# o1-labs/proof-systems

Hardware: AMD Instinct MI355X
Metric: MSM Mscalar/s at 2^20 (Vesta) (higher is better)
Workload: dtype u29x9 / u32x8 (255-bit Montgomery integers); 1 GPU; msm_2^20_vesta_srs; points_per_gpu=1048576, points_total=1048576, bases=SRS::<Vesta>::create, scalars=uniform 254-bit, seed 1234+rank, parallelism=point-range x1, world_size_seen=1

## Files before the change

proof_systems_amd/csrc/msm.hip:

```cpp
#include <hip/hip_ext.h>
#include <math.h>
#include "common.hpp"
#include "env.hpp"
#include "curve.cuh"
#include "coop.cuh"
#include "field29.cuh"
#include "host_ec.hpp"
#include "msm.hpp"
#include <condition_variable>
#include <functional>
#include <memory>
#include <thread>

namespace kh {

#define KH_HIGH_PRIO() __builtin_amdgcn_s_setprio(3)

class HostHelper {
    std::thread th_; std::mutex m_; std::condition_variable cv_, done_cv_;
    std::function<void()> job_; bool has_job_ = false, busy_ = false, stop_ = false;
    void loop() {
        std::unique_lock<std::mutex> lk(m_);
        for (;;) {
            cv_.wait(lk, [&] { return has_job_ || stop_; });
// ... 328 lines not shown
        for (int u = 0; u < 8; u++) {
            const u32 b = (u32)(v[u] < 0 ? -v[u] : v[u]) - 1u;
            const u32 pos = lds_inc_agg(cur, b >> PART_LOW, v[u] != 0);
            if (v[u]) mid[pos] = ((b & ((1u << PART_LOW) - 1u)) << 25) | (v[u] < 0 ? 1u << 24 : 0u) | (w << 20) | i;
            i += PART_T;
            while (i >= n) { i -= n; w++; }
        }
    }
}
__global__ void __launch_bounds__(PART_T)
k_part_sort(const u32* __restrict__ mid, const u32* __restrict__ PO, u32 nblk, u32 nb, size_t pt_stride, size_t pt_offset, size_t pt_batch,
            u32 last_group, u32* __restrict__ off, u32* __restrict__ entries) {
    KH_HIGH_PRIO();
    __shared__ u32 hist[1u << PART_LOW], cur[1u << PART_LOW];
    const u32 pidx = blockIdx.x, j = blockIdx.y, tid = threadIdx.x;
    const size_t q = (size_t)j * PART_P + pidx;
    const u32 base = PO[q * nblk], end = PO[(q + 1) * nblk];
    if (tid < (1u << PART_LOW)) hist[tid] = 0;
    __syncthreads();
    for (u32 x0 = base + tid; x0 < end; x0 += 8 * PART_T) {
        u32 m[8];
#pragma unroll
        for (int u = 0; u < 8; u++) { const u32 x = x0 + u * PART_T; m[u] = mid[x < end ? x : end - 1]; }
#pragma unroll
        for (int u = 0; u < 8; u++) (void)lds_inc_agg(hist, m[u] >> 25, x0 + u * PART_T < end);
    }
    __syncthreads();
    if (tid < 64) {
        const u32 a = hist[2 * tid], b = hist[2 * tid + 1];
        u32 inc = a + b;
#pragma unroll
        for (int d = 1; d < 64; d <<= 1) { const u32 o = __shfl_up(inc, d, 64); if (tid >= (u32)d) inc += o; }
        const u32 ex = base + inc - (a + b);
        u32* o = off + (size_t)j * nb + (size_t)pidx * (1u << PART_LOW);
        o[2 * tid] = ex; o[2 * tid + 1] = ex + a;
        cur[2 * tid] = ex; cur[2 * tid + 1] = ex + a;
        if (tid == 63 && pidx == PART_P - 1 && j == last_group) off[(size_t)(j + 1) * nb] = end;
    }
    __syncthreads();
    const u32 pb0 = (u32)(pt_offset + (size_t)j * pt_batch);
    for (u32 x0 = base + tid; x0 < end; x0 += 8 * PART_T) {
        u32 m[8];
#pragma unroll
        for (int u = 0; u < 8; u++) { const u32 x = x0 + u * PART_T; m[u] = mid[x < end ? x : end - 1]; }
#pragma unroll
        for (int u = 0; u < 8; u++) {
            const bool live = x0 + u * PART_T < end;
            const u32 pos = lds_inc_agg(cur, m[u] >> 25, live);
            if (live) entries[pos] = (pb0 + (u32)(((m[u] >> 20) & 15u) * pt_stride) + (m[u] & 0xfffffu)) | ((m[u] & (1u << 24)) << 7);
        }
    }
}
static constexpr u32 MAX_K = 256;
struct KTab { uint8_t k[48]; };
__device__ __forceinline__ u32 pick_K(u32 total, u32 room, u32 kmin, const KTab& tab, u32 nkeys) {
    u32 K = (total + room - 1) / room;
    u32 lo = kmin;
    if (total && nkeys) {
        const float m = (float)total / (float)nkeys;
        int idx = (int)(4.0f * __log2f(m) + 8.5f);
        idx = idx < 0 ? 0 : (idx > 47 ? 47 : idx);
        if (tab.k[idx]) lo = tab.k[idx];
    }
    return K < lo ? lo : (K > MAX_K ? MAX_K : K);
}
__global__ void k_task_reset(u32* __restrict__ len_hist, u32* __restrict__ big) {
    KH_HIGH_PRIO();
    if (threadIdx.x <= MAX_K) len_hist[threadIdx.x] = 0;
    if (threadIdx.x < 2) big[threadIdx.x] = 0;
}
__global__ void k_ntask(const u32* __restrict__ off, size_t nkeys, u32 room, u32 kmin, KTab ktab, u32* __restrict__ nt, u32* __restrict__ len_hist, u32* __restrict__ handed) {
    KH_HIGH_PRIO();
    __shared__ u32 h[MAX_K + 1];
    if (handed && blockIdx.x == 0 && threadIdx.x == 0) handed[0] = 0;
    for (u32 i = threadIdx.x; i <= MAX_K; i += blockDim.x) h[i] = 0;
    __syncthreads();
    const u32 K = pick_K(off[nkeys], room, kmin, ktab, (u32)nkeys);
    size_t key = (size_t)blockIdx.x * blockDim.x + threadIdx.x;
    if (key <= nkeys) {
        u32 n_t = 0;
        if (key < nkeys) {
            u32 c = off[key + 1] - off[key];
            n_t = (c + K - 1) / K;
            u32 len = n_t ? (c + n_t - 1) / n_t : 0;
            atomicAdd(&h[len], 1u);
        }
        nt[key] = n_t;
    }
    __syncthreads();
    for (u32 i = threadIdx.x; i <= MAX_K; i += blockDim.x) if (h[i]) atomicAdd(&len_hist[i], h[i]);
}
__global__ void __launch_bounds__(320) k_len_starts(const u32* __restrict__ len_hist, u32* __restrict__ cursor) {
    KH_HIGH_PRIO();
    __shared__ u32 h[MAX_K + 1];
    if (threadIdx.x <= MAX_K) h[threadIdx.x] = len_hist[threadIdx.x];
    __syncthreads();
    if (threadIdx.x <= MAX_K) {
        u32 run = 0;
        for (u32 L = threadIdx.x + 1; L <= MAX_K; L++) run += h[L];
        cursor[threadIdx.x] = run;
    }
}
__global__ void __launch_bounds__(1024)
k_len_rank(const u32* __restrict__ off, const u32* __restrict__ nt, size_t nkeys,
           u32* __restrict__ cursor, u32* __restrict__ order, u32* __restrict__ rnt) {
    KH_HIGH_PRIO();
// ... 173 lines not shown
    if (!grid_barrier(sync, 3 * G, abort_dev, abort_host, spin_limit)) return;
    KH_TS(6);
    const u32* o = off + (size_t)j * g.nb + b_lo;
    {
        u32 a[FUSED_C], hh[FUSED_C];
#pragma unroll
        for (int u = 0; u < FUSED_C; u++) { const u32 b = tid + u * FUSED_T, bc = b < g.sub ? b : 0u; a[u] = coh_load(o + bc); hh[u] = coh_load(hout + bc); }
        u32 total2;
        lane_sums(bsums + FUSED_B, G, blk, &base, &total2);
#pragma unroll
        for (int u = 0; u < FUSED_C; u++) { const u32 b = tid + u * FUSED_T; if (b < g.sub) lds[b] = a[u] + hh[u]; }
    }
    run = base + ex2;
#pragma unroll
    for (int i = 0; i < FUSED_KPT; i++) {
        const u32 key = key0 + i;
        if ((u32)i < g.kpt && key <= g.nkeys) toff[key] = run;
        run += nt[i];
    }
    __syncthreads();
    KH_TS(7);
    const u32 pb0 = (u32)(g.pt_offset + (size_t)j * g.pt_batch);
    const u32 e_first = 4 * (q_lo + tid);
    u32 w = e_first / g.n, i = e_first - w * g.n;
#pragma unroll
    for (int t = 0; t < FUSED_V; t++) asm volatile("" : "+v"(dv[t][0]), "+v"(dv[t][1]));
#pragma unroll
    for (int t = 0; t < FUSED_V; t++) {
#pragma unroll
        for (int l = 0; l < 4; l++) {
            const u32 c = (dv[t][l >> 1] >> (16 * (l & 1))) & 0xffffu, b = (c & 0x7fffu) - b_lo;
            if (c != 0xffffu && b < g.sub) {
                u32 ii = i + l, ww = w;
                if (ii >= g.n) { ii -= g.n; ww++; }
                const u32 slot = atomicAdd(&lds[b], 1u);
                entries[slot] = (pb0 + (u32)(ww * g.pt_stride) + ii) | ((c & 0x8000u) << 16);
            }
        }
        i += 4 * FUSED_T;
        while (i >= g.n) { i -= g.n; w++; }
    }
    __syncthreads();
    KH_TS(8);
    if (tid == 0) {
        const u32 out = __hip_atomic_fetch_add(sync + 1, 1u, __ATOMIC_RELAXED, __HIP_MEMORY_SCOPE_AGENT);
        if (out == G - 1) {
            __hip_atomic_store(sync, 0u, __ATOMIC_RELAXED, __HIP_MEMORY_SCOPE_AGENT);
            __hip_atomic_store(sync + 1, 0u, __ATOMIC_RELAXED, __HIP_MEMORY_SCOPE_AGENT);
        }
    }
}
static constexpr u32 PART2_MAXLOW = 11, PART2_MAXPASS = 8;
__global__ void __launch_bounds__(PART_T)
k_part2_scatter(const int32_t* __restrict__ digits, u32 tot_e, u32 nblk, u32 low, const u32* __restrict__ PO, u32* __restrict__ mid, u32* __restrict__ xlist, u32* __restrict__ big) {
    KH_HIGH_PRIO();
    __shared__ u32 cur[PART_P];
    const u32 blk = blockIdx.x, j = blockIdx.y, tid = threadIdx.x;
    if (blk == 0 && j == 0 && tid == 0) { xlist[0] = 0; xlist[1] = 0; big[0] = 0; }
    if (tid < PART_P) cur[tid] = PO[((size_t)j * PART_P + tid) * nblk + blk];
    __syncthreads();
    const u32 e_lo = (u32)((u64)tot_e * blk / nblk), e_hi = (u32)((u64)tot_e * (blk + 1) / nblk);
    const int32_t* d = digits + (size_t)j * tot_e;
    for (u32 e0 = e_lo + tid; e0 < e_hi; e0 += 8 * PART_T) {
        int32_t v[8];
#pragma unroll
        for (int u = 0; u < 8; u++) { const u32 e = e0 + u * PART_T; v[u] = d[e < e_hi ? e : e_hi - 1]; if (e >= e_hi) v[u] = 0; }
#pragma unroll
        for (int u = 0; u < 8; u++) {
            const u32 b = (u32)(v[u] < 0 ? -v[u] : v[u]) - 1u;
            const u32 pos = lds_inc_agg(cur, b & (PART_P - 1u), v[u] != 0);
            if (v[u]) mid[pos] = ((b >> 8) << 17) | (v[u] < 0 ? 1u << 16 : 0u) | (e0 + u * PART_T - e_lo);
        }
    }
}
struct WideTasks { u32 room, kmin, nkeys; KTab ktab; };
__global__ void __launch_bounds__(PART_T)
k_part2_sort(const u32* __restrict__ mid, const u32* __restrict__ PO, u32 nblk, u32 low, u32 nb, u32 tot_e, u32 n, size_t pt_stride, size_t pt_offset,
             size_t pt_batch, u32 last_group, size_t total_idx, WideTasks ta, u32* __restrict__ off, u32* __restrict__ entries,
             u32* __restrict__ toff, u32* __restrict__ order, u32* __restrict__ ptot, u32* __restrict__ xlist, u32* __restrict__ slist,
             uint8_t* __restrict__ buckets29, u32 og, u32 stage_cap, u32 max_pass, u32* __restrict__ big, u32 bigcap, u32 hot_nt) {
    KH_HIGH_PRIO();
    __shared__ u32 cur[1u << PART2_MAXLOW], pstart[1025], bi0[1024], bw0[1024], lh[MAX_K + 2], sh[PART_T / 64 + 1];
    __shared__ u32 xl_n, pfirst[PART2_MAXPASS], plast[PART2_MAXPASS];
    extern __shared__ u32 stage[];
    u32* const xl_key = stage; u32* const xl_nt = stage + (1u << PART2_MAXLOW); u32* const xl_base = stage + (2u << PART2_MAXLOW);
    const u32 pidx = blockIdx.x, j = blockIdx.y, tid = threadIdx.x;
    const size_t q = (size_t)j * PART_P + pidx;
    const u32 nparts = gridDim.x * gridDim.y;
    const u32 nbl = 1u << low;
    for (u32 i = tid; i <= nblk; i += PART_T) pstart[i] = PO[q * nblk + i];
    for (u32 i = tid; i < nblk; i += PART_T) {
        const u32 est = (u32)((u64)tot_e * i / nblk), w0 = est / n;
        bw0[i] = w0; bi0[i] = est - w0 * n;
    }
    for (u32 i = tid; i < nbl; i += PART_T) cur[i] = 0;
    for (u32 i = tid; i < MAX_K + 2; i += PART_T) lh[i] = 0;
    if (tid == 0) xl_n = 0;
    __syncthreads();
    const u32 base = pstart[0], end = pstart[nblk];
    for (u32 x0 = base + tid; x0 < end; x0 += 8 * PART_T) {
        u32 m[8];
#pragma unroll
        for (int u = 0; u < 8; u++) { const u32 x = x0 + u * PART_T; m[u] = mid[x < end ? x : end - 1]; }
#pragma unroll
        for (int u = 0; u < 8; u++) (void)lds_inc_agg(cur, m[u] >> 17, x0 + u * PART_T < end);
    }
    __syncthreads();
    {
        const u32 i0 = 2 * tid, a = i0 < nbl ? cur[i0] : 0u, b = i0 + 1 < nbl ? cur[i0 + 1] : 0u;
        u32 btot;
        const u32 ex = base + block_scan_1024(a + b, sh, &btot);
        __syncthreads();
        const size_t key0 = (size_t)j * nb + (size_t)pidx * nbl + i0;
        if (i0 < nbl) { off[key0] = ex; cur[i0] = ex; }
        if (i0 + 1 < nbl) { off[key0 + 1] = ex + a; cur[i0 + 1] = ex + a; }
        if (tid == 0 && pidx == PART_P - 1 && j == last_group) off[(size_t)(j + 1) * nb] = end;
        const u32 K = pick_K(PO[total_idx], ta.room, ta.kmin, ta.ktab, ta.nkeys);
        const u32 nta = (a + K - 1) / K, ntb = (b + K - 1) / K;
        const u32 la = nta ? (a + nta - 1) / nta : 0u, lb = ntb ? (b + ntb - 1) / ntb : 0u;
        const u32 tex = block_scan_1024(nta + ntb, sh, &btot);
        if (i0 < nbl) toff[key0] = tex;
        if (i0 + 1 < nbl) toff[key0 + 1] = tex + nta;
        if (tid == 0) ptot[q] = btot;
        if (i0 < nbl) atomicAdd(&lh[la], 1u);
        if (i0 + 1 < nbl) atomicAdd(&lh[lb], 1u);
        if (nta > 1) { const u32 sl = atomicAdd(&xl_n, 1u); xl_key[sl] = (u32)key0; xl_nt[sl] = nta; xl_base[sl] = atomicAdd(&xlist[0], nta - 1u); slist[atomicAdd(&xlist[1], 1u)] = (u32)key0; }
        if (ntb > 1) { const u32 sl = atomicAdd(&xl_n, 1u); xl_key[sl] = (u32)key0 + 1u; xl_nt[sl] = ntb; xl_base[sl] = atomicAdd(&xlist[0], ntb - 1u); slist[atomicAdd(&xlist[1], 1u)] = (u32)key0 + 1u; }
        if (nta > hot_nt) { const u32 sl = atomicAdd(&big[0], 1u); big[2 + sl] = (u32)key0; big[2 + bigcap + sl] = 0u; }
        if (ntb > hot_nt) { const u32 sl = atomicAdd(&big[0], 1u); big[2 + sl] = (u32)key0 + 1u; big[2 + bigcap + sl] = 0u; }
        if (i0 < nbl && a == 0) { uint4* rec = (uint4*)(buckets29 + ((size_t)j * nb + ((size_t)i0 << 8 | pidx)) * B29_BYTES); _Pragma("unroll") for (int t = 0; t < 9; t++) rec[t] = make_uint4(0u, 0u, 0u, 0u); }
        if (i0 + 1 < nbl && b == 0) { uint4* rec = (uint4*)(buckets29 + ((size_t)j * nb + ((size_t)(i0 + 1) << 8 | pidx)) * B29_BYTES); _Pragma("unroll") for (int t = 0; t < 9; t++) rec[t] = make_uint4(0u, 0u, 0u, 0u); }
        __syncthreads();
        const u32 L = MAX_K - (tid <= MAX_K ? tid : MAX_K), hv = tid <= MAX_K ? lh[L] : 0u;
        const u32 above = block_scan_1024(hv, sh, &btot);
        __syncthreads();
        if (tid <= MAX_K) lh[L] = above;
        __syncthreads();
        if (i0 < nbl) { const u32 r = atomicAdd(&lh[la], 1u); order[(size_t)(r / og) * nparts * og + q * og + (r % og)] = (u32)key0; }
        if (i0 + 1 < nbl) { const u32 r = atomicAdd(&lh[lb], 1u); order[(size_t)(r / og) * nparts * og + q * og + (r % og)] = (u32)key0 + 1u; }
        const u32 nx = xl_n;
        for (u32 it = 0; it < nx; it++) {
            const u32 key = xl_key[it], ntx = xl_nt[it], xb = xl_base[it];
            for (u32 jt = 1 + tid; jt < ntx; jt += PART_T) { xlist[2 + 2 * (size_t)(xb + jt - 1)] = key; xlist[3 + 2 * (size_t)(xb + jt - 1)] = jt; }
        }
    }
    __syncthreads();
    const u32 pb0 = (u32)(pt_offset + (size_t)j * pt_batch);
    const u32 lane = tid & 63u, wv = tid >> 6;
    const u32 S_eff = stage_cap > 2048u ? stage_cap - 1024u : 0u;
    const u32 npass = S_eff ? (end - base + S_eff - 1u) / S_eff : 0u;
    const bool staged = S_eff != 0u && npass >= 1u && npass <= max_pass;
    uint8_t* const bpass = (uint8_t*)(stage + stage_cap);
    if (staged) {
        if (tid < PART2_MAXPASS) { pfirst[tid] = 0xffffffffu; plast[tid] = 0u; }
        __syncthreads();
        for (u32 b = tid; b < nbl; b += PART_T) {
            const u32 o = cur[b], oe = b + 1 < nbl ? cur[b + 1] : end, pb = (o - base) / S_eff;
            bpass[b] = (uint8_t)pb;
            if (oe > o) { atomicMin(&pfirst[pb], o); atomicMax(&plast[pb], oe); }
        }
        __syncthreads();
    }
    for (u32 pass = 0; pass < (staged ? npass : 1u); pass++) {
        const u32 p0 = staged ? pfirst[pass] : 0u, p1 = staged ? plast[pass] : 0u;
        if (staged && p0 == 0xffffffffu) continue;
        for (u32 blk = wv; blk < nblk; blk += PART_T / 64) {
            const u32 rs = pstart[blk], re = pstart[blk + 1];
            const u32 w0 = bw0[blk], i0 = bi0[blk];
            for (u32 x0 = rs; x0 < re; x0 += 256) {
                u32 m[4];
#pragma unroll
                for (int u = 0; u < 4; u++) { const u32 x = x0 + u * 64 + lane; m[u] = mid[x < re ? x : re - 1]; }
#pragma unroll
                for (int u = 0; u < 4; u++) {
                    if (x0 + u * 64 >= re) break;
                    const u32 bk = m[u] >> 17;
                    const bool live = x0 + u * 64 + lane < re && (!staged || bpass[bk] == pass);
                    const u32 pos = lds_inc_agg(cur, bk, live);
                    if (live) {
                        u32 w = w0, i = i0 + (m[u] & 0xffffu);
                        while (i >= n) { i -= n; w++; }
                        const u32 val = (pb0 + (u32)(w * pt_stride) + i) | ((m[u] & (1u << 16)) << 15);
                        if (staged && pos - p0 < stage_cap) stage[pos - p0] = val;
                        else entries[pos] = val;
                    }
                }
            }
        }
        if (staged) {
            __syncthreads();
            const u32 cnt = p1 - p0 < stage_cap ? p1 - p0 : stage_cap;
            for (u32 k = tid; k < cnt; k += PART_T) entries[p0 + k] = stage[k];
            __syncthreads();
        }
    }
}
__global__ void __launch_bounds__(256)
k_wide_fixup(u32* __restrict__ toff, const u32* __restrict__ ptot, u32 nparts, u32 low, u32 nkeys, u32* __restrict__ handed, u32* __restrict__ big) {
    KH_HIGH_PRIO();
    __shared__ u32 sh[4];
    const u32 key = blockIdx.x * 256 + threadIdx.x, q = (blockIdx.x * 256) >> low;
    u32 v = 0;
    for (u32 t = threadIdx.x; t < q && t < nparts; t += 256) v += ptot[t];
#pragma unroll
    for (int d = 32; d >= 1; d >>= 1) v += __shfl_xor(v, d, 64);
    if ((threadIdx.x & 63u) == 0) sh[threadIdx.x >> 6] = v;
    __syncthreads();
    const u32 bs = sh[0] + sh[1] + sh[2] + sh[3];
    if (key < nkeys) toff[key] += bs;
    else if (key == nkeys) toff[key] = bs;
    if (key == 0) handed[0] = 0;
}
template <class BF>
__global__ void __launch_bounds__(256) __attribute__((amdgpu_num_vgpr(112), amdgpu_waves_per_eu(4, 4)))
k_accumulate29(const u32* __restrict__ entries, const u32* __restrict__ off, const u32* __restrict__ toff,
               const u32* __restrict__ roff, const u32* __restrict__ order,
               size_t nkeys, const uint8_t* __restrict__ pts, uint8_t* __restrict__ partial, u32* __restrict__ handed, const u32* __restrict__ abort_dev, u32 hi_prio) {
    if (hi_prio) __builtin_amdgcn_s_setprio(2);
    if (sort_gave_up(abort_dev)) return;
    const size_t t0 = (size_t)blockIdx.x * blockDim.x + threadIdx.x;
    u32 NT = roff[nkeys];
    if (t0 >= NT) return;
    size_t lo = 0, hi = nkeys;
    while (hi - lo > 1) {
        size_t mid = (lo + hi) >> 1;
        if (roff[mid] <= (u32)t0) lo = mid; else hi = mid;
    }
    size_t key = order ? order[lo] : lo;
    u32 jt = (u32)t0 - roff[lo];
    const size_t t = (size_t)toff[key] + jt;
    u32 o0 = off[key], cnt = off[key + 1] - o0, nt = toff[key + 1] - toff[key];
    u32 start = o0 + (u32)(((u64)jt * cnt) / nt);
    u32 end = o0 + (u32)(((u64)(jt + 1) * cnt) / nt);
    u32 e = entries[start];
    Aff<BF> p = Aff<BF>::load(pts + (size_t)(e & 0x7fffffffu) * 64);
    if (e >> 31) p.y = neg<BF>(p.y);
    typedef typename C29<BF>::T K29;
    Acc29<BF> acc;
    acc.x = to29<BF>(p.x); acc.y = to29<BF>(p.y);
#pragma unroll
    for (int i = 0; i < 9; i++) { acc.zz.v[i] = K29::one(i); acc.zzz.v[i] = K29::one(i); }
    bool ok = true;
    for (u32 k = start + 1; k < end; k++) {
        e = entries[k];
        p = Aff<BF>::load(pts + (size_t)(e & 0x7fffffffu) * 64);
        if (e >> 31) p.y = neg<BF>(p.y);
        ok = madd29<BF>(acc, pack29<BF, 5>(p.x), pack29<BF, 5>(p.y));
        if (!ok) break;
    }
    Xyzz<BF> r;
    if (__builtin_expect(!ok, 0)) {
        e = entries[start];
        p = Aff<BF>::load(pts + (size_t)(e & 0x7fffffffu) * 64);
        if (e >> 31) p.y = neg<BF>(p.y);
        r = Xyzz<BF>::from_affine(p);
        for (u32 k = start + 1; k < end; k++) {
            e = entries[k];
            p = Aff<BF>::load(pts + (size_t)(e & 0x7fffffffu) * 64);
            r = madd<BF>(r, p, (e >> 31) != 0);
        }
    } else {
        r.x = from29<BF>(acc.x); r.y = from29<BF>(acc.y); r.zz = from29<BF>(acc.zz); r.zzz = from29<BF>(acc.zzz);
    }
    r.store(partial + t * 128);
// ... 507 lines not shown
        if (!have) { acc = b; have = true; ok = !is_marker29<BF>(b); }
        else ok = !is_marker29<BF>(b) && add29<BF>(acc, b);
        if (!ok) break;
    }
    if (!ok) { acc.zz.v[0] = 0xffffffffu; store_b29<BF>(o, acc); return; }
    if (have) store_b29<BF>(o, acc); else store_b29_identity<BF>(o);
}
template <class BF>
__global__ void __launch_bounds__(256)
k_wide_a1(const uint8_t* __restrict__ buckets29, WideGeom g, u32 ngroups, uint8_t* __restrict__ out29) {
    KH_HIGH_PRIO();
    const u32 per = g.nb >> g.rlog, items = 2u * per;
    const u32 gid = blockIdx.x * blockDim.x + threadIdx.x;
    if (gid >= items * ngroups) return;
    const u32 q = gid / items, u = gid - q * items;
    u32 out = u;
    if (u >= per) { const u32 v = u - per, b = v & ((1u << g.lo) - 1u), sc = v >> g.lo; out = per + b * ((1u << g.hi) >> g.rlog) + sc; }
    u32 t0, ts;
    wide_a1_item(g, out, t0, ts);
    wide_sum29<BF>(buckets29 + ((size_t)q * g.nb + t0) * B29_BYTES, (size_t)ts * B29_BYTES, 1u << g.rlog, out29 + ((size_t)q * items + out) * B29_BYTES);
}
template <class BF>
__global__ void __launch_bounds__(256)
k_wide_l2(const uint8_t* __restrict__ in29, u32 flog, u32 nrec, uint8_t* __restrict__ out29) {
    KH_HIGH_PRIO();
    const u32 gid = blockIdx.x * blockDim.x + threadIdx.x;
    if (gid >= nrec) return;
    wide_sum29<BF>(in29 + ((size_t)gid << flog) * B29_BYTES, B29_BYTES, 1u << flog, out29 + (size_t)gid * B29_BYTES);
}
template <class BF>
__device__ __attribute__((noinline)) Xyzz<BF> wide_chunk_exact(const uint8_t* __restrict__ buckets29g, WideGeom g, u32 out) {
    u32 t0, ts;
    wide_a1_item(g, out, t0, ts);
    Xyzz<BF> acc = Xyzz<BF>::identity();
    const u32 r = 1u << g.rlog;
    for (u32 i = 0; i < r; i++) {
        const Acc29<BF> b = load_b29<BF>(buckets29g + ((size_t)t0 + (size_t)i * ts) * B29_BYTES);
        if (!is_identity29<BF>(b)) acc = add<BF>(acc, xyzz_from29<BF>(b));
    }
    return acc;
}
template <class BF>
__device__ __attribute__((noinline)) Xyzz<BF> wide_run_exact(const uint8_t* __restrict__ chunks29g, const uint8_t* __restrict__ buckets29g, WideGeom g, u32 run) {
    Xyzz<BF> acc = Xyzz<BF>::identity();
    const u32 f = 1u << g.flog, c0 = run << g.flog;
    for (u32 i = 0; i < f; i++) {
        const Acc29<BF> b = load_b29<BF>(chunks29g + (size_t)(c0 + i) * B29_BYTES);
        if (is_marker29<BF>(b)) acc = add<BF>(acc, wide_chunk_exact<BF>(buckets29g, g, c0 + i));
        else if (!is_identity29<BF>(b)) acc = add<BF>(acc, xyzz_from29<BF>(b));
    }
    return acc;
}
template <class BF>
__global__ void __launch_bounds__(64)
k_wide_a2(const uint8_t* __restrict__ runs29, const uint8_t* __restrict__ chunks29, const uint8_t* __restrict__ buckets29, WideGeom g, uint8_t* __restrict__ outw) {
    KH_HIGH_PRIO();
    __shared__ u32 stage[32][16];
    const u32 q = blockIdx.y, lane = threadIdx.x, role = lane & 3u, quad = lane >> 2;
    const u32 per = g.nb >> g.rlog, per2 = per >> g.flog;
    const u32 r0 = blockIdx.x * 16u, plane = r0 >= per2 ? 1u : 0u;
    const u32 s = ((1u << (plane ? g.hi : g.lo)) >> g.rlog) >> g.flog;
    uint8_t* const og = outw + ((size_t)q * 2 + plane) * (1u << g.lo) * 128;
    if (lane < 16) {
        const u32 run = r0 + lane;
        const Acc29<BF> b = load_b29<BF>(runs29 + ((size_t)q * 2 * per2 + run) * B29_BYTES);
        Xyzz<BF> a = Xyzz<BF>::identity();
        if (__builtin_expect(is_marker29<BF>(b), 0)) a = wide_run_exact<BF>(chunks29 + (size_t)q * 2 * per * B29_BYTES, buckets29 + (size_t)q * g.nb * B29_BYTES, g, run);
        else if (!is_identity29<BF>(b)) a = xyzz_from29<BF>(b);
#pragma unroll
        for (int k = 0; k < 8; k++) { stage[k][lane] = a.x.v[k]; stage[8 + k][lane] = a.y.v[k]; stage[16 + k][lane] = a.zz.v[k]; stage[24 + k][lane] = a.zzz.v[k]; }
    }
    __syncthreads();
    Fe<BF> acc;
#pragma unroll
    for (int k = 0; k < 8; k++) acc.v[k] = stage[role * 8 + k][quad];
    for (u32 d = s >> 1; d >= 1; d >>= 1) acc = quad_add<BF>(acc, quad_shfl_down<BF>(acc, (int)d));
    if ((quad & (s - 1u)) == 0u) {
        const u32 m = (r0 - plane * per2 + quad) / s;
        if (plane || m) quad_store<BF>(og + (size_t)(m - (plane ? 0u : 1u)) * 128, acc);
    }
    if (plane == 0 && lane < 4)
        for (u32 p = (1u << g.hi) - 1u + blockIdx.x; p < (1u << g.lo); p += per2 / 16u) quad_store<BF>(og + (size_t)p * 128, Fe<BF>::zero());
}

template <class BF>
__global__ void __launch_bounds__(256)
k_precompute(uint8_t* __restrict__ tables, const uint8_t* __restrict__ inf, size_t n, int c, int W, uint8_t* __restrict__ scratch) {
    size_t i = (size_t)blockIdx.x * blockDim.x + threadIdx.x;
    if (i >= n) return;
    if (inf && inf[i]) {
        for (int w = 1; w < W; w++) { Fe<BF> z = Fe<BF>::zero(); z.store(tables + ((size_t)w * n + i) * 64); z.store(tables + ((size_t)w * n + i) * 64 + 32); }
        return;
    }
    Xyzz<BF> P = Xyzz<BF>::from_affine(Aff<BF>::load(tables + i * 64));
    Fe<BF> prod = Fe<BF>::one();
    for (int w = 1; w < W; w++) {
        for (int k = 0; k < c; k++) P = dbl<BF>(P);
        P.store(scratch + ((size_t)(w - 1) * n + i) * 128);
        prod = mul<BF>(prod, P.zzz);
        prod.store(tables + ((size_t)w * n + i) * 64);
    }
    Fe<BF> iv = inv<BF>(prod);
    for (int w = W - 1; w >= 1; w--) {
        Xyzz<BF> Q = Xyzz<BF>::load(scratch + ((size_t)(w - 1) * n + i) * 128);
        Fe<BF> izzz = iv;
        if (w > 1) izzz = mul<BF>(iv, Fe<BF>::load(tables + ((size_t)(w - 1) * n + i) * 64));
        iv = mul<BF>(iv, Q.zzz);
        Fe<BF> izz = sqr<BF>(mul<BF>(izzz, Q.zz));
        Fe<BF> x = mul<BF>(Q.x, izz), y = mul<BF>(Q.y, izzz);
        x.store(tables + ((size_t)w * n + i) * 64);
        y.store(tables + ((size_t)w * n + i) * 64 + 32);
    }
}

struct VestaCfg { typedef FqParams Base; typedef FpParams Scalar; };
struct PallasCfg { typedef FpParams Base; typedef FqParams Scalar; };

static std::atomic<size_t>& wide_min_n_cell() {
    static std::atomic<size_t> v{(size_t)env_int("KH_WIDE_MIN_N", 1 << 19)};
    return v;
}
static std::atomic<u32>& sort_staging_cell(int i) {
    static std::atomic<u32> v[2] = {{(u32)env_int("KH_PART2_STAGE", 28672)}, {(u32)env_int("KH_PART2_MAXPASS", 2)}};
    return v[i];
}
void msm_set_sort_staging(unsigned entries, unsigned max_passes) { sort_staging_cell(0).store(entries); sort_staging_cell(1).store(max_passes); }
size_t msm_wide_min_n() { const size_t v = wide_min_n_cell().load(); return v ? v : ~(size_t)0; }
void msm_set_wide_min_n(size_t n) { wide_min_n_cell().store(n); }
// ... 32 lines not shown
    return t;
}

template <class CFG>
static int msm_enqueue_t(Context& Ctx, MsmSlot& C, const MsmBasis& basis, size_t offset, const u64* scalars_dev, size_t n, size_t k,
                         int mont, int curve, int flags) {
    typedef typename CFG::Base BF; typedef typename CFG::Scalar SF;
    hipStream_t s = C.stream;
    const bool wide = basis.wide_pts && basis.wide_c > 16 && basis.wide_c - 9 <= (int)PART2_MAXLOW && n >= msm_wide_min_n() && k <= 4 &&
                      (size_t)windows_of(basis.wide_c) * n <= ((size_t)1 << 26);
    static constexpr u32 SPREAD_MAX_NT = 256;
    const void* const tab_pts = wide ? basis.wide_pts : basis.pts;
    const int c = wide ? basis.wide_c : (basis.precomp_c ? basis.precomp_c : msm_pick_window(n));
    const bool glv = basis.glv && !wide && basis.precomp_c != 0;
    const int W = glv ? 2 * ((128 + c - 1) / c) : windows_of(c);
    const u32 nb = 1u << (c - 1);
    const int precomp = (wide || basis.precomp_c) ? 1 : 0;
    int S = (int)(n / 32768); if (S < 1) S = 1; if (S > 16) S = 16;
    { int want = (int)(512 / ((size_t)W * k)); if (want < 1) want = 1; if (S > want) S = want; }
    const size_t tab_stride = basis.stride ? basis.stride : basis.n;
    SortGeom g{n, nb, S, W, precomp, tab_stride, offset, basis.batch_stride};
    const size_t ngroups = precomp ? k : k * (size_t)W;
    const bool few_groups = ngroups <= 8;
    const bool quad_sum = !wide && precomp && few_groups;
    const bool spread = quad_sum && (flags & MSM_SPREAD_SCALARS) != 0;
    const int Sq = precomp ? W * S : S;
    const size_t nkeys = ngroups * nb;
    const size_t M = n * (size_t)W * k;
    const size_t cap = (size_t)Ctx.num_cus * 256 * 4;
    size_t room_sz = cap / 4;
    if (nkeys < cap / 2) room_sz = cap - cap / 16 - nkeys / 2;
    const u32 room = (u32)room_sz;
    const u32 kmin = 8;
    const KTab ktab = precomp ? task_length_table(nkeys, (u32)Ctx.num_cus) : KTab{};
    const size_t max_tasks = M / 4 + nkeys + 1;
    KH_REQUIRE(M < ((size_t)1 << 31) && (tab_stride * (size_t)(precomp ? W : 1) + basis.batch_stride * k) < ((size_t)1 << 31), "MSM too large for 31-bit entry indices (n=%zu k=%zu)", n, k);

    int rc;
    if ((rc = C.ws_digits.reserve(M * sizeof(int32_t)))) return rc;
    if ((rc = C.ws_hist.reserve(nkeys * Sq * sizeof(u32)))) return rc;
    if ((rc = C.ws_cnt.reserve((nkeys + 2) * sizeof(u32)))) return rc;
    if ((rc = C.ws_off.reserve((nkeys + 2) * sizeof(u32)))) return rc;
    if ((rc = C.ws_ntask.reserve((nkeys + 2) * sizeof(u32)))) return rc;
    if ((rc = C.ws_toff.reserve((nkeys + 2) * sizeof(u32)))) return rc;
    if ((rc = C.ws_entries.reserve((M + 1) * sizeof(u32)))) return rc;
    if ((rc = C.ws_partial.reserve(max_tasks * 128))) return rc;
    if ((rc = C.ws_handed.reserve((max_tasks + 2) * sizeof(u32)))) return rc;
    if ((rc = C.ws_buckets.reserve(nkeys * 128))) return rc;
    const size_t bigcap = nkeys + max_tasks / CHUNK + 2;
    if ((rc = C.ws_biglist.reserve((2 + 4 * bigcap) * sizeof(u32)))) return rc;
    if ((rc = C.ws_chunks.reserve(bigcap * 128))) return rc;
    if ((rc = C.ws_order.reserve((2 * (MAX_K + 1) + 3 * (nkeys + 2)) * sizeof(u32)))) return rc;
    WideGeom wg{};
    static constexpr u32 wide_og = 16, wide_acc_blocks = 3, wide_rlog = 4;
    static_assert((wide_og & (wide_og - 1)) == 0 && wide_og <= (1u << (17 - 9)) && wide_rlog >= 1 && wide_rlog + 2 <= 17 / 2, "wide-path constants");
    size_t wide_acc_lds = (Ctx.lds_per_cu / (wide_acc_blocks + 1) + 1024) & ~(size_t)1023;
    if (wide_acc_lds > Ctx.lds_per_block) wide_acc_lds = Ctx.lds_per_block & ~(size_t)1023;
    if (wide) {
        if ((rc = C.ws_xlist.reserve((3 * max_tasks + 8) * sizeof(u32)))) return rc;
        if ((rc = C.ws_handed.reserve((2 * max_tasks + 4) * sizeof(u32)))) return rc;
        wg.nb = nb; wg.lo = (u32)c / 2; wg.hi = (u32)(c - 1) - wg.lo; wg.rlog = wide_rlog;
        wg.flog = wg.lo > wg.rlog + 5 ? wg.lo - wg.rlog - 4 : 1;
        if ((rc = C.ws_b29.reserve(nkeys * B29_BYTES))) return rc;
        if ((rc = C.ws_a1.reserve(ngroups * 2 * (size_t)(nb >> wg.rlog) * B29_BYTES))) return rc;
        if ((rc = C.ws_l2.reserve(ngroups * 2 * (size_t)(nb >> (wg.rlog + wg.flog)) * B29_BYTES))) return rc;
        if ((rc = C.ws_a2.reserve(ngroups * 2 * ((size_t)1 << wg.lo) * 128))) return rc;
    }
    u32 m = 1;
    while (m < 16 && (ngroups * (size_t)nb) / m > 65536) m <<= 1;
    if (!precomp && m < 4) m = 4;
    if (nb < m) m = nb;
    const u32 nseg = nb / m;
    const u32 nblk1 = (nseg + SUM_BLK - 1) / SUM_BLK;
    const u32 planes = wide ? 3u : ((precomp && ngroups <= 4096 && c >= 7 && c <= 16) ? 3u : 0u);
    MargGeom mg{};
    if (planes) {
        const u32 bits = wide ? wg.lo : (u32)c - 1, f0 = (bits + 2) / 3, f1 = (bits - f0 + 1) / 2, f2 = bits - f0 - f1;
        mg.nb = wide ? 1u << wg.lo : nb; mg.sh[0] = 0; mg.wd[0] = f0; mg.sh[1] = f0; mg.wd[1] = f1; mg.sh[2] = f0 + f1; mg.wd[2] = f2;
    }
    const size_t tail_groups = wide ? 2 * ngroups : ngroups;
    const size_t nout = planes ? tail_groups * planes : ngroups;
    if ((rc = C.ws_seg.reserve(std::max(ngroups * (size_t)(nseg + nblk1), nout * (size_t)32) * 128))) return rc;
    if ((rc = C.ws_out.reserve(nout * 128))) return rc;
    if (C.pinned_cap < nout * 128) {
        if (C.pinned) (void)hipHostFree(C.pinned);
        C.pinned = nullptr; C.pinned_cap = 0;
        C.pinned_coherent = hipHostMalloc(&C.pinned, nout * 128 + 4096, hipHostMallocCoherent | hipHostMallocMapped) == hipSuccess;
        if (!C.pinned_coherent) { (void)hipGetLastError(); C.pinned = nullptr; KH_HIP(hipHostMalloc(&C.pinned, nout * 128 + 4096, hipHostMallocDefault)); }
        C.pinned_cap = nout * 128 + 4096;
    }
    if (Ctx.once("msm_attr")) {
        KH_HIP(hipFuncSetAttribute((const void*)k_hist, hipFuncAttributeMaxDynamicSharedMemorySize, 131072));
        KH_HIP(hipFuncSetAttribute((const void*)k_scatter, hipFuncAttributeMaxDynamicSharedMemorySize, 131072));
        KH_HIP(hipFuncSetAttribute((const void*)k_sort_fused, hipFuncAttributeMaxDynamicSharedMemorySize, 131072));
    }
    static const bool fused_off = env_flag("KH_NO_FUSED_SORT", false);
    static const unsigned long long fused_spin_ticks = 100ull * (unsigned long long)env_int("KH_FUSED_SPIN_US", 20000);
    FusedGeom fg{};
    bool fused = precomp && !wide && !fused_off && !Ctx.fused_disabled && k <= 4 && M < ((size_t)1 << 22) && nb >= 2048 && Ctx.num_cus >= 128;
    if (fused) {
        fg.n = (u32)n; fg.nb = nb; fg.W = (u32)W; fg.k = (u32)k; fg.bpg = (u32)std::min<size_t>(FUSED_G, FUSED_B / (2 * k)); fg.nkeys = (u32)nkeys;
        fg.split = 2; fg.sub = nb / fg.split;
        fg.room = room; fg.kmin = kmin; fg.ktab = ktab; fg.pt_stride = tab_stride; fg.pt_offset = offset; fg.pt_batch = basis.batch_stride;
        const size_t threads = (size_t)fg.bpg * k * fg.split * FUSED_T;
        fg.kpt = (u32)((nkeys + 1 + threads - 1) / threads);
        const size_t tot4 = (size_t)W * n / 4, chunk4 = (tot4 + fg.bpg - 1) / fg.bpg + 1;
        if (fg.kpt > (u32)FUSED_KPT || n < 4 || ((size_t)W * n) % 4 || chunk4 > (size_t)FUSED_V * FUSED_T || fg.sub > (u32)FUSED_C * FUSED_T) fused = false;
    }
// ... 14 lines not shown
            KH_HIP(hipMemsetAsync(C.ws_sync.p, 0, (2 + 2 * FUSED_B + 32 + 2) * sizeof(u32), s));
        }
        if (!C.host_abort) {
            void* hp = nullptr;
            KH_HIP(hipHostMalloc(&hp, 64, hipHostMallocCoherent | hipHostMallocMapped));
            C.host_abort = (volatile uint32_t*)hp; *C.host_abort = 0;
        }
    }
    if (spread && !C.spread_abort) {
        void* hp = nullptr;
        KH_HIP(hipHostMalloc(&hp, 64, hipHostMallocCoherent | hipHostMallocMapped));
        C.spread_abort = (volatile uint32_t*)hp; *C.spread_abort = 0;
    }
    static const bool flag_off = env_flag("KH_NO_DONE_FLAG", false);
    bool flag_on = !flag_off && (wide || planes) && !C.flag_unavailable && C.pinned_coherent;
    if (flag_on && !C.done_flag) {
        void* hp = nullptr;
        if (hipHostMalloc(&hp, 64, hipHostMallocCoherent | hipHostMallocMapped) != hipSuccess) {
            (void)hipGetLastError(); C.flag_unavailable = true; flag_on = false;
        } else {
            C.done_flag = (volatile uint32_t*)hp; *C.done_flag = 0; C.done_expect = 0;
            if ((rc = C.ws_done.reserve(64))) return rc;
            KH_HIP(hipMemsetAsync(C.ws_done.p, 0, 64, s));
        }
    }
    C.timer.begin(s);
    if (glv)
    hipLaunchKernelGGL((k_digits_glv<SF>), dim3((unsigned)((n + 255) / 256), (unsigned)k), dim3(256), 0, s,
                       scalars_dev, basis.inf, offset, basis.batch_stride, n, mont, c, W, C.ws_digits.as<int32_t>());
    else
    hipLaunchKernelGGL((k_digits<SF>), dim3((unsigned)((n + 255) / 256), (unsigned)k), dim3(256), 0, s,
                       scalars_dev, basis.inf, offset, basis.batch_stride, n, mont, c, W, C.ws_digits.as<int32_t>(), (size_t)0, n);
    C.timer.mark("digits", s);
    u32* len_hist = C.ws_order.as<u32>();
    u32* cursor = len_hist + (MAX_K + 1);
    u32* order = cursor + (MAX_K + 1);
    u32* rnt = order + (nkeys + 2);
    u32* roff = rnt + (nkeys + 2);
    if (fused) {
        order = nullptr; roff = C.ws_toff.as<u32>();
        u32* sy = C.ws_sync.as<u32>();
        hipLaunchKernelGGL(k_sort_fused, dim3(fg.bpg * fg.k * fg.split), dim3(FUSED_T), (size_t)fg.sub * sizeof(u32), s, C.ws_digits.as<int32_t>(), fg,
                           C.ws_hist.as<u32>(), C.ws_off.as<u32>(), C.ws_toff.as<u32>(), C.ws_entries.as<u32>(), C.ws_handed.as<u32>(),
                           C.ws_biglist.as<u32>(), sy, sy + 2, C.host_abort, fused_spin_ticks);
        C.timer.mark("sort", s);
    } else if (part) {
        const u32 tot_e = (u32)((size_t)W * n);
        const dim3 pgrid(part_nblk, (unsigned)k);
        hipLaunchKernelGGL(k_part_hist, pgrid, dim3(PART_T), 0, s, C.ws_digits.as<int32_t>(), tot_e, part_nblk, wide ? 0u : part_low, C.ws_hist.as<u32>());
        C.timer.mark("histogram", s);
        if ((rc = exclusive_scan_u32(C.ws_hist.as<u32>(), C.ws_cnt.as<u32>(), part_size + 1, C.ws_scan_tmp, s))) return rc;
        C.timer.mark("scan", s);
        if (wide) {
            hipLaunchKernelGGL(k_part2_scatter, pgrid, dim3(PART_T), 0, s, C.ws_digits.as<int32_t>(), tot_e, part_nblk, part_low, C.ws_cnt.as<u32>(), C.ws_mid.as<u32>(), C.ws_xlist.as<u32>(), C.ws_biglist.as<u32>());
            const WideTasks wt{room, kmin, (u32)nkeys, ktab};
            u32* const slist = C.ws_xlist.as<u32>() + 2 + 2 * max_tasks;
            u32* const ptot = C.ws_ntask.as<u32>();
            const u32 part2_stage = sort_staging_cell(0).load(), part2_maxpass = std::min<u32>(PART2_MAXPASS, sort_staging_cell(1).load());
            u32 stage_now = std::min<u32>(part2_stage, (131072u - (1u << PART2_MAXLOW)) / 4u);
            if (stage_now <= 2048u || (size_t)W * n / PART_P > (size_t)part2_maxpass * (stage_now - 1024u)) stage_now = 0;
            const u32 stage_words = std::max<u32>(stage_now, 3u << PART2_MAXLOW);
            const size_t part2_lds = (size_t)stage_words * 4 + (stage_now ? ((size_t)1 << PART2_MAXLOW) : 0);
            if (Ctx.once("part2_attr")) KH_HIP(hipFuncSetAttribute((const void*)k_part2_sort, hipFuncAttributeMaxDynamicSharedMemorySize, 131072));
            hipLaunchKernelGGL(k_part2_sort, dim3(PART_P, (unsigned)k), dim3(PART_T), part2_lds, s, C.ws_mid.as<u32>(), C.ws_cnt.as<u32>(), part_nblk, part_low, nb, tot_e, (u32)n,
                               tab_stride, offset, basis.batch_stride, (u32)(k - 1), part_size, wt, C.ws_off.as<u32>(), C.ws_entries.as<u32>(),
                               C.ws_toff.as<u32>(), order, ptot, C.ws_xlist.as<u32>(), slist, C.ws_b29.as<uint8_t>(), wide_og, stage_now, part2_maxpass, C.ws_biglist.as<u32>(), (u32)bigcap, WIDE_HOT_NT);
            hipLaunchKernelGGL(k_wide_fixup, dim3((unsigned)(nkeys / 256 + 1)), dim3(256), 0, s, C.ws_toff.as<u32>(), ptot, (u32)(k * PART_P), part_low, (u32)nkeys,
                               C.ws_handed.as<u32>(), C.ws_biglist.as<u32>());
        } else {
        hipLaunchKernelGGL(k_part_scatter, pgrid, dim3(PART_T), 0, s, C.ws_digits.as<int32_t>(), tot_e, (u32)n, part_nblk, C.ws_cnt.as<u32>(), C.ws_mid.as<u32>());
        hipLaunchKernelGGL(k_part_sort, dim3(PART_P, (unsigned)k), dim3(PART_T), 0, s, C.ws_mid.as<u32>(), C.ws_cnt.as<u32>(), part_nblk, nb,
                           tab_stride, offset, basis.batch_stride, (u32)(k - 1), C.ws_off.as<u32>(), C.ws_entries.as<u32>());
        }
        C.timer.mark("scatter", s);
    } else {
        size_t lds = (size_t)nb * sizeof(u32);
        dim3 sgrid((unsigned)S, (unsigned)W, (unsigned)k);
        hipLaunchKernelGGL(k_hist, sgrid, dim3(1024), lds, s, C.ws_digits.as<int32_t>(), g, C.ws_hist.as<u32>());
        hipLaunchKernelGGL(k_key_totals, dim3((unsigned)((nkeys + 1 + 255) / 256)), dim3(256), 0, s,
                           C.ws_hist.as<u32>(), nb, Sq, nkeys, C.ws_cnt.as<u32>());
        C.timer.mark("histogram", s);
        if ((rc = exclusive_scan_u32(C.ws_cnt.as<u32>(), C.ws_off.as<u32>(), nkeys + 1, C.ws_scan_tmp, s))) return rc;
        C.timer.mark("scan", s);
        hipLaunchKernelGGL(k_scatter, sgrid, dim3(1024), lds, s, C.ws_digits.as<int32_t>(), g, C.ws_hist.as<u32>(),
                           C.ws_off.as<u32>(), C.ws_entries.as<u32>());
        C.timer.mark("scatter", s);
    }
    if (!fused && !wide) {
        hipLaunchKernelGGL(k_task_reset, dim3(1), dim3(320), 0, s, len_hist, C.ws_biglist.as<u32>());
        hipLaunchKernelGGL(k_ntask, dim3((unsigned)((nkeys + 1 + 1023) / 1024)), dim3(1024), 0, s, C.ws_off.as<u32>(), nkeys, room, kmin, ktab, C.ws_ntask.as<u32>(), len_hist, C.ws_handed.as<u32>());
        if ((rc = exclusive_scan_u32(C.ws_ntask.as<u32>(), C.ws_toff.as<u32>(), nkeys + 1, C.ws_scan_tmp, s))) return rc;
        if (M >= ((size_t)1 << 22)) {
            hipLaunchKernelGGL(k_len_starts, dim3(1), dim3(320), 0, s, len_hist, cursor);
            hipLaunchKernelGGL(k_len_rank, dim3((unsigned)((nkeys + 1 + 1023) / 1024)), dim3(1024), 0, s, C.ws_off.as<u32>(), C.ws_ntask.as<u32>(), nkeys, cursor, order, rnt);
            if ((rc = exclusive_scan_u32(rnt, roff, nkeys + 1, C.ws_scan_tmp, s))) return rc;
        } else {
            order = nullptr; roff = C.ws_toff.as<u32>();
        }
        C.timer.mark("tasks", s);
    }
    const u32* abort_dev = fused ? C.ws_sync.as<u32>() + 2 + 2 * FUSED_B + 32 : nullptr;
    const dim3 agrid((unsigned)((max_tasks + 255) / 256));
    const u32 acc_prio = (flags & MSM_LATENCY) ? 1u : 0u;
    uint8_t* const b29 = wide ? C.ws_b29.as<uint8_t>() : nullptr;
    if (wide) {
        const dim3 wgrid((unsigned)(nkeys / 256));
        auto kern = k_acc_wide29<BF>;
        if (C.timer.enabled && C.timer.created) {
            hipExtLaunchKernelGGL(kern, wgrid, dim3(256), wide_acc_lds, s, C.timer.k0, C.timer.k1, 0, C.ws_entries.as<u32>(), C.ws_off.as<u32>(), C.ws_toff.as<u32>(), order, (u32)nkeys,
                                  (const uint8_t*)tab_pts, C.ws_partial.as<uint8_t>(), b29, part_low, C.ws_handed.as<u32>());
            C.timer.kname = "k_acc_wide29";
        } else
        hipLaunchKernelGGL(kern, wgrid, dim3(256), wide_acc_lds, s, C.ws_entries.as<u32>(), C.ws_off.as<u32>(), C.ws_toff.as<u32>(), order, (u32)nkeys,
                           (const uint8_t*)tab_pts, C.ws_partial.as<uint8_t>(), b29, part_low, C.ws_handed.as<u32>());
        const unsigned xgrid = M / nkeys >= 64 ? 2048u : WIDE_XB;
        hipLaunchKernelGGL((k_acc_wide_rest<BF>), dim3(xgrid), dim3(256), 0, s, C.ws_entries.as<u32>(), C.ws_off.as<u32>(), C.ws_toff.as<u32>(), C.ws_xlist.as<u32>(),
                           C.ws_handed.as<u32>(), (const uint8_t*)tab_pts, C.ws_partial.as<uint8_t>(), b29, part_low);
    } else {
        auto kern = k_accumulate29<BF>;
        if (C.timer.enabled && C.timer.created) {
            hipExtLaunchKernelGGL(kern, agrid, dim3(256), 0, s, C.timer.k0, C.timer.k1, 0,
// ... 287 lines not shown
```

Baseline: 1064 Mscalar/s.

## Build a global length-sorted bucket order and lane-parallelise wide run loading

The per-partition interleaved bucket order (og-strided by length rank) is replaced with a globally length-sorted order. Per-block length histograms are atomically merged into global totals, each key's place is recorded, and k_wide_fixup scans the totals and scatters the keys. Separately, k_wide_a2 now loads run records directly per quad lane instead of staging through LDS, and handles marker runs through a ballot-guarded quad helper. This is meant to improve load balance in later bucket processing and cut LDS staging and sync, at the cost of extra global atomics and a scan in the fixup kernel.

```diff
diff --git a/proof_systems_amd/csrc/msm.hip b/proof_systems_amd/csrc/msm.hip
--- a/proof_systems_amd/csrc/msm.hip
+++ b/proof_systems_amd/csrc/msm.hip
@@ -404,6 +404,8 @@
     }
 }
 static constexpr u32 MAX_K = 256;
+static constexpr u32 LEN_CLASSES = MAX_K + 1;
+static_assert(MAX_K == 256, "k_wide_fixup scans the length classes with its 256 threads");
 struct KTab { uint8_t k[48]; };
 __device__ __forceinline__ u32 pick_K(u32 total, u32 room, u32 kmin, const KTab& tab, u32 nkeys) {
     u32 K = (total + room - 1) / room;
@@ -683,11 +685,13 @@
 }
 static constexpr u32 PART2_MAXLOW = 11, PART2_MAXPASS = 8;
 __global__ void __launch_bounds__(PART_T)
-k_part2_scatter(const int32_t* __restrict__ digits, u32 tot_e, u32 nblk, u32 low, const u32* __restrict__ PO, u32* __restrict__ mid, u32* __restrict__ xlist, u32* __restrict__ big) {
+k_part2_scatter(const int32_t* __restrict__ digits, u32 tot_e, u32 nblk, u32 low, const u32* __restrict__ PO, u32* __restrict__ mid, u32* __restrict__ xlist, u32* __restrict__ big,
+                u32* __restrict__ ltot) {
     KH_HIGH_PRIO();
     __shared__ u32 cur[PART_P];
     const u32 blk = blockIdx.x, j = blockIdx.y, tid = threadIdx.x;
     if (blk == 0 && j == 0 && tid == 0) { xlist[0] = 0; xlist[1] = 0; big[0] = 0; }
+    if (blk == 0 && j == 0 && tid < LEN_CLASSES) ltot[tid] = 0;
     if (tid < PART_P) cur[tid] = PO[((size_t)j * PART_P + tid) * nblk + blk];
     __syncthreads();
     const u32 e_lo = (u32)((u64)tot_e * blk / nblk), e_hi = (u32)((u64)tot_e * (blk + 1) / nblk);
@@ -708,8 +712,8 @@
 __global__ void __launch_bounds__(PART_T)
 k_part2_sort(const u32* __restrict__ mid, const u32* __restrict__ PO, u32 nblk, u32 low, u32 nb, u32 tot_e, u32 n, size_t pt_stride, size_t pt_offset,
              size_t pt_batch, u32 last_group, size_t total_idx, WideTasks ta, u32* __restrict__ off, u32* __restrict__ entries,
-             u32* __restrict__ toff, u32* __restrict__ order, u32* __restrict__ ptot, u32* __restrict__ xlist, u32* __restrict__ slist,
-             uint8_t* __restrict__ buckets29, u32 og, u32 stage_cap, u32 max_pass, u32* __restrict__ big, u32 bigcap, u32 hot_nt) {
+             u32* __restrict__ toff, uint2* __restrict__ lplace, u32* ltot, u32* __restrict__ ptot,
+             u32* __restrict__ xlist, u32* __restrict__ slist, uint8_t* __restrict__ buckets29, u32 stage_cap, u32 max_pass, u32* __restrict__ big, u32 bigcap, u32 hot_nt) {
     KH_HIGH_PRIO();
     __shared__ u32 cur[1u << PART2_MAXLOW], pstart[1025], bi0[1024], bw0[1024], lh[MAX_K + 2], sh[PART_T / 64 + 1];
     __shared__ u32 xl_n, pfirst[PART2_MAXPASS], plast[PART2_MAXPASS];
@@ -717,7 +721,6 @@
     u32* const xl_key = stage; u32* const xl_nt = stage + (1u << PART2_MAXLOW); u32* const xl_base = stage + (2u << PART2_MAXLOW);
     const u32 pidx = blockIdx.x, j = blockIdx.y, tid = threadIdx.x;
     const size_t q = (size_t)j * PART_P + pidx;
-    const u32 nparts = gridDim.x * gridDim.y;
     const u32 nbl = 1u << low;
     for (u32 i = tid; i <= nblk; i += PART_T) pstart[i] = PO[q * nblk + i];
     for (u32 i = tid; i < nblk; i += PART_T) {
@@ -762,13 +765,12 @@
         if (i0 < nbl && a == 0) { uint4* rec = (uint4*)(buckets29 + ((size_t)j * nb + ((size_t)i0 << 8 | pidx)) * B29_BYTES); _Pragma("unroll") for (int t = 0; t < 9; t++) rec[t] = make_uint4(0u, 0u, 0u, 0u); }
         if (i0 + 1 < nbl && b == 0) { uint4* rec = (uint4*)(buckets29 + ((size_t)j * nb + ((size_t)(i0 + 1) << 8 | pidx)) * B29_BYTES); _Pragma("unroll") for (int t = 0; t < 9; t++) rec[t] = make_uint4(0u, 0u, 0u, 0u); }
         __syncthreads();
-        const u32 L = MAX_K - (tid <= MAX_K ? tid : MAX_K), hv = tid <= MAX_K ? lh[L] : 0u;
-        const u32 above = block_scan_1024(hv, sh, &btot);
+        if (tid <= MAX_K) { const u32 hv = lh[tid]; lh[tid] = hv ? atomicAdd(&ltot[tid], hv) : 0u; }
         __syncthreads();
-        if (tid <= MAX_K) lh[L] = above;
-        __syncthreads();
-        if (i0 < nbl) { const u32 r = atomicAdd(&lh[la], 1u); order[(size_t)(r / og) * nparts * og + q * og + (r % og)] = (u32)key0; }
-        if (i0 + 1 < nbl) { const u32 r = atomicAdd(&lh[lb], 1u); order[(size_t)(r / og) * nparts * og + q * og + (r % og)] = (u32)key0 + 1u; }
+        if (i0 < nbl) {
+            const u32 pa = atomicAdd(&lh[la], 1u), pb = atomicAdd(&lh[lb], 1u);
+            *(uint4*)(lplace + key0) = make_uint4(pa, la, pb, lb);
+        }
         const u32 nx = xl_n;
         for (u32 it = 0; it < nx; it++) {
             const u32 key = xl_key[it], ntx = xl_nt[it], xb = xl_base[it];
@@ -827,9 +829,10 @@
     }
 }
 __global__ void __launch_bounds__(256)
-k_wide_fixup(u32* __restrict__ toff, const u32* __restrict__ ptot, u32 nparts, u32 low, u32 nkeys, u32* __restrict__ handed, u32* __restrict__ big) {
-    KH_HIGH_PRIO();
-    __shared__ u32 sh[4];
+k_wide_fixup(u32* __restrict__ toff, const u32* __restrict__ ptot, u32 nparts, u32 low, u32 nkeys, u32* __restrict__ handed, u32* __restrict__ big,
+             const uint2* __restrict__ lplace, const u32* __restrict__ ltot, u32* __restrict__ order) {
+    KH_HIGH_PRIO();
+    __shared__ u32 sh[4], first[LEN_CLASSES], wsum[4];
     const u32 key = blockIdx.x * 256 + threadIdx.x, q = (blockIdx.x * 256) >> low;
     u32 v = 0;
     for (u32 t = threadIdx.x; t < q && t < nparts; t += 256) v += ptot[t];
@@ -841,6 +844,19 @@
     if (key < nkeys) toff[key] += bs;
     else if (key == nkeys) toff[key] = bs;
     if (key == 0) handed[0] = 0;
+    if (q >= nparts) return;
+    const uint2 pl = lplace[key];
+    const u32 tid = threadIdx.x, lane = tid & 63u, c = ltot[MAX_K - tid];
+    u32 inc = c;
+#pragma unroll
+    for (int d = 1; d < 64; d <<= 1) { const u32 o = __shfl_up(inc, d, 64); if (lane >= (u32)d) inc += o; }
+    if (lane == 63) wsum[tid >> 6] = inc;
+    __syncthreads();
+    for (u32 w2 = 0; w2 < (tid >> 6); w2++) inc += wsum[w2];
+    first[MAX_K - tid] = inc - c;
+    if (tid == 255) first[0] = inc;
+    __syncthreads();
+    order[first[pl.y] + pl.x] = key;
 }
 template <class BF>
 __global__ void __launch_bounds__(256) __attribute__((amdgpu_num_vgpr(112), amdgpu_waves_per_eu(4, 4)))
@@ -1454,28 +1470,40 @@
     return acc;
 }
 template <class BF>
+__device__ __attribute__((noinline)) Fe<BF> wide_run_exact_quad(const uint8_t* __restrict__ chunks29g, const uint8_t* __restrict__ buckets29g, WideGeom g, u32 run, bool marked, Fe<BF> cur) {
+    const u32 lane = threadIdx.x & 63u, role = lane & 3u;
+    Xyzz<BF> ex = Xyzz<BF>::identity();
+    if (marked && role == 0u) ex = wide_run_exact<BF>(chunks29g, buckets29g, g, run);
+    const int src = (int)(lane & ~3u);
+#pragma unroll
+    for (int k = 0; k < 8; k++) {
+        const u32 x = __shfl(ex.x.v[k], src, 64), y = __shfl(ex.y.v[k], src, 64), zz = __shfl(ex.zz.v[k], src, 64), zzz = __shfl(ex.zzz.v[k], src, 64);
+        if (marked) cur.v[k] = role == 0u ? x : role == 1u ? y : role == 2u ? zz : zzz;
+    }
+    return cur;
+}
+template <class BF>
 __global__ void __launch_bounds__(64)
 k_wide_a2(const uint8_t* __restrict__ runs29, const uint8_t* __restrict__ chunks29, const uint8_t* __restrict__ buckets29, WideGeom g, uint8_t* __restrict__ outw) {
     KH_HIGH_PRIO();
-    __shared__ u32 stage[32][16];
     const u32 q = blockIdx.y, lane = threadIdx.x, role = lane & 3u, quad = lane >> 2;
     const u32 per = g.nb >> g.rlog, per2 = per >> g.flog;
     const u32 r0 = blockIdx.x * 16u, plane = r0 >= per2 ? 1u : 0u;
     const u32 s = ((1u << (plane ? g.hi : g.lo)) >> g.rlog) >> g.flog;
     uint8_t* const og = outw + ((size_t)q * 2 + plane) * (1u << g.lo) * 128;
-    if (lane < 16) {
-        const u32 run = r0 + lane;
-        const Acc29<BF> b = load_b29<BF>(runs29 + ((size_t)q * 2 * per2 + run) * B29_BYTES);
-        Xyzz<BF> a = Xyzz<BF>::identity();
-        if (__builtin_expect(is_marker29<BF>(b), 0)) a = wide_run_exact<BF>(chunks29 + (size_t)q * 2 * per * B29_BYTES, buckets29 + (size_t)q * g.nb * B29_BYTES, g, run);
-        else if (!is_identity29<BF>(b)) a = xyzz_from29<BF>(b);
-#pragma unroll
-        for (int k = 0; k < 8; k++) { stage[k][lane] = a.x.v[k]; stage[8 + k][lane] = a.y.v[k]; stage[16 + k][lane] = a.zz.v[k]; stage[24 + k][lane] = a.zzz.v[k]; }
-    }
-    __syncthreads();
-    Fe<BF> acc;
-#pragma unroll
-    for (int k = 0; k < 8; k++) acc.v[k] = stage[role * 8 + k][quad];
+    const u32 run = r0 + quad;
+    const u32* const limbs = (const u32*)(runs29 + ((size_t)q * 2 * per2 + run) * B29_BYTES) + role * 9u;
+    Fe29<BF> c;
+#pragma unroll
+    for (int i = 0; i < 9; i++) c.v[i] = limbs[i];
+    u32 any = 0;
+#pragma unroll
+    for (int i = 0; i < 9; i++) any |= c.v[i];
+    const u32 kind = __shfl((any == 0u ? 1u : 0u) | (c.v[0] == 0xffffffffu ? 2u : 0u), (int)((lane & ~3u) | 2u), 64);
+    Fe<BF> acc = Fe<BF>::zero();
+    if (kind == 0u) acc = from29<BF>(c);
+    if (__builtin_expect(__ballot(kind & 2u) != 0ull, 0))
+        acc = wide_run_exact_quad<BF>(chunks29 + (size_t)q * 2 * per * B29_BYTES, buckets29 + (size_t)q * g.nb * B29_BYTES, g, run, (kind & 2u) != 0u, acc);
     for (u32 d = s >> 1; d >= 1; d >>= 1) acc = quad_add<BF>(acc, quad_shfl_down<BF>(acc, (int)d));
     if ((quad & (s - 1u)) == 0u) {
         const u32 m = (r0 - plane * per2 + quad) / s;
@@ -1614,8 +1642,8 @@
     if ((rc = C.ws_chunks.reserve(bigcap * 128))) return rc;
     if ((rc = C.ws_order.reserve((2 * (MAX_K + 1) + 3 * (nkeys + 2)) * sizeof(u32)))) return rc;
     WideGeom wg{};
-    static constexpr u32 wide_og = 16, wide_acc_blocks = 3, wide_rlog = 4;
-    static_assert((wide_og & (wide_og - 1)) == 0 && wide_og <= (1u << (17 - 9)) && wide_rlog >= 1 && wide_rlog + 2 <= 17 / 2, "wide-path constants");
+    static constexpr u32 wide_acc_blocks = 3, wide_rlog = 4;
+    static_assert(256u <= (1u << (17 - 9)) && wide_rlog >= 1 && wide_rlog + 2 <= 17 / 2, "wide-path constants");
     size_t wide_acc_lds = (Ctx.lds_per_cu / (wide_acc_blocks + 1) + 1024) & ~(size_t)1023;
     if (wide_acc_lds > Ctx.lds_per_block) wide_acc_lds = Ctx.lds_per_block & ~(size_t)1023;
     if (wide) {
@@ -1736,7 +1764,8 @@
         if ((rc = exclusive_scan_u32(C.ws_hist.as<u32>(), C.ws_cnt.as<u32>(), part_size + 1, C.ws_scan_tmp, s))) return rc;
         C.timer.mark("scan", s);
         if (wide) {
-            hipLaunchKernelGGL(k_part2_scatter, pgrid, dim3(PART_T), 0, s, C.ws_digits.as<int32_t>(), tot_e, part_nblk, part_low, C.ws_cnt.as<u32>(), C.ws_mid.as<u32>(), C.ws_xlist.as<u32>(), C.ws_biglist.as<u32>());
+            hipLaunchKernelGGL(k_part2_scatter, pgrid, dim3(PART_T), 0, s, C.ws_digits.as<int32_t>(), tot_e, part_nblk, part_low, C.ws_cnt.as<u32>(), C.ws_mid.as<u32>(), C.ws_xlist.as<u32>(), C.ws_biglist.as<u32>(), len_hist);
+            uint2* const lplace = (uint2*)rnt;
             const WideTasks wt{room, kmin, (u32)nkeys, ktab};
             u32* const slist = C.ws_xlist.as<u32>() + 2 + 2 * max_tasks;
             u32* const ptot = C.ws_ntask.as<u32>();
@@ -1748,9 +1777,9 @@
             if (Ctx.once("part2_attr")) KH_HIP(hipFuncSetAttribute((const void*)k_part2_sort, hipFuncAttributeMaxDynamicSharedMemorySize, 131072));
             hipLaunchKernelGGL(k_part2_sort, dim3(PART_P, (unsigned)k), dim3(PART_T), part2_lds, s, C.ws_mid.as<u32>(), C.ws_cnt.as<u32>(), part_nblk, part_low, nb, tot_e, (u32)n,
                                tab_stride, offset, basis.batch_stride, (u32)(k - 1), part_size, wt, C.ws_off.as<u32>(), C.ws_entries.as<u32>(),
-                               C.ws_toff.as<u32>(), order, ptot, C.ws_xlist.as<u32>(), slist, C.ws_b29.as<uint8_t>(), wide_og, stage_now, part2_maxpass, C.ws_biglist.as<u32>(), (u32)bigcap, WIDE_HOT_NT);
+                               C.ws_toff.as<u32>(), lplace, len_hist, ptot, C.ws_xlist.as<u32>(), slist, C.ws_b29.as<uint8_t>(), stage_now, part2_maxpass, C.ws_biglist.as<u32>(), (u32)bigcap, WIDE_HOT_NT);
             hipLaunchKernelGGL(k_wide_fixup, dim3((unsigned)(nkeys / 256 + 1)), dim3(256), 0, s, C.ws_toff.as<u32>(), ptot, (u32)(k * PART_P), part_low, (u32)nkeys,
-                               C.ws_handed.as<u32>(), C.ws_biglist.as<u32>());
+                               C.ws_handed.as<u32>(), C.ws_biglist.as<u32>(), lplace, len_hist, order);
         } else {
         hipLaunchKernelGGL(k_part_scatter, pgrid, dim3(PART_T), 0, s, C.ws_digits.as<int32_t>(), tot_e, (u32)n, part_nblk, C.ws_cnt.as<u32>(), C.ws_mid.as<u32>());
         hipLaunchKernelGGL(k_part_sort, dim3(PART_P, (unsigned)k), dim3(PART_T), 0, s, C.ws_mid.as<u32>(), C.ws_cnt.as<u32>(), part_nblk, nb,
```

After: 1067 Mscalar/s, median of 6. Within noise of the previous version (+0.3%).
